# Sidharthshanu/Gossip-protocol-with-power-law

Measured on AMD Instinct MI355X. Metric: gossip edge-deliveries/s (GTEPS) & HBM roofline %, 2^24 nodes x 4096 msgs, higher is better.
Workload: dtype u64

## Files before the change

### gossip-protocol-with-power-law_amd/csrc/driver.hip

```cpp
#include <hip/hip_runtime.h>

#include <cstdlib>
#include <rccl/rccl.h>

#include <algorithm>
#include <cmath>
#include <cstring>
#include <string>
#include <vector>

#include "gp_device.h"
#include "xplan.h"

namespace gp {

static thread_local std::string g_err;
int set_error(int code, const std::string& msg) {
  g_err = msg;
  return code;
}
int copy_sync(Ctx* c, void* dst, const void* src, size_t bytes, hipMemcpyKind kind) {
  if (bytes == 0) return 0;
  GP_HIP(hipMemcpyAsync(dst, src, bytes, kind, c->stream));
  GP_HIP(hipStreamSynchronize(c->stream));
  return 0;
}

__global__ void k_stats_reduce(u64* __restrict__ partial, u64* __restrict__ stats) {
  __shared__ u64 acc[BLOCK];
  const int k = blockIdx.x;
  u64 t = 0;
  for (int p = threadIdx.x; p < NPART; p += BLOCK) {
    t += partial[(size_t)k * NPART + p];
    partial[(size_t)k * NPART + p] = 0;
  }
  acc[threadIdx.x] = t;
  __syncthreads();
  for (int w = BLOCK / 2; w > 0; w >>= 1) {
    if (threadIdx.x < w) acc[threadIdx.x] += acc[threadIdx.x + w];
    __syncthreads();
  }
  if (threadIdx.x == 0) stats[k] += acc[0];
}

__global__ __launch_bounds__(BLOCK) void k_mkbits(const uint32_t* __restrict__ fpop, u64* __restrict__ abits,
                                                  int64_t n, const uint32_t* __restrict__ seenpop,
                                                  const uint32_t* __restrict__ done_at, u64* __restrict__ dbits,
                                                  const uint8_t* __restrict__ sated,
                                                  const int32_t* __restrict__ deg_live, u64* __restrict__ partial) {
  const int lane = threadIdx.x & 63;
  const int64_t stride = (int64_t)gridDim.x * BLOCK;
  u64 sends = 0, active = 0;
  for (int64_t v0 = (int64_t)blockIdx.x * BLOCK + (threadIdx.x & ~63); v0 < n; v0 += stride) {
    const int64_t v = v0 + lane;
    const uint32_t fp = v < n ? fpop[v] : 0u;
    const u64 m = __ballot(fp != 0u);
    if (deg_live && fp) {
      sends += (u64)fp * (u64)(uint32_t)max(deg_live[v], 0);
      ++active;
    }
    if (lane == 0) abits[v0 >> 6] = m;
    if (dbits) {
      bool d = false;
      if (v < n) {
        if (sated) {
          const uint8_t sv = sated[v];
          const uint32_t t = done_at[v];
          d = !(sv & ST_DOWN) && ((sv & ST_SATED) || (t != 0u && seenpop[v] == t));
        } else {
          const uint32_t t = done_at[v];
          d = t != 0u && seenpop[v] == t;
        }
      }
      const u64 dm = __ballot(d);
      if (lane == 0) dbits[v0 >> 6] = dm;
    }
  }
  if (deg_live) {
    sends = wave_sum_u64(sends);
    active = wave_sum_u64(active);
    if (lane == 0) {
      const size_t p = blockIdx.x % NPART;
      if (sends) atomicAdd(&partial[(size_t)S_SENDS * NPART + p], sends);
      if (active) atomicAdd(&partial[(size_t)S_ACTIVE * NPART + p], active);
    }
  }
}

__global__ __launch_bounds__(BLOCK) void k_mksum(const u64* __restrict__ abits, u64* __restrict__ sbits,
                                                 int64_t nwords) {
  const int lane = threadIdx.x & 63;
  const int64_t k = (int64_t)blockIdx.x * WAVES + (threadIdx.x >> 6);
  const int64_t w = k * 64 + lane;
  const u64 m = __ballot(w < nwords && abits[w] != 0ull);
  if (lane == 0 && k * 64 < nwords) sbits[k] = m;
}

__global__ void k_lost_clear(const int32_t* __restrict__ origin, const u64* __restrict__ bits,
                             const uint32_t* __restrict__ cnt, const uint8_t* __restrict__ state,
                             const int32_t* __restrict__ midx, u64* __restrict__ cmask,
                             uint32_t* __restrict__ lostcnt, int64_t off, int64_t groups, int32_t words) {
  const int64_t t = (int64_t)blockIdx.x * blockDim.x + threadIdx.x;
  if (t >= groups * words) return;
  const int64_t gi = off + t / words;
  const int32_t w = (int32_t)(t % words);
  const int32_t o = origin[gi];
  if (!(state[o] & ST_DOWN)) return;
  const int32_t k = midx[o];
  atomicAnd(cmask + (size_t)k * words + w, ~bits[gi * words + w]);
  if (w == 0) atomicAdd(lostcnt + k, cnt[gi]);
}
__global__ void k_done_fix(const int32_t* __restrict__ midx, const uint32_t* __restrict__ lostcnt,
                           uint32_t* __restrict__ done_at, int64_t n) {
  for (int64_t v = (int64_t)blockIdx.x * blockDim.x + threadIdx.x; v < n; v += (int64_t)gridDim.x * blockDim.x) {
    const int32_t k = midx[v];
    if (k >= 0) {
      const uint32_t l = lostcnt[k];
      if (l) done_at[v] -= l;
    }
  }
}

struct InjectArgs {
  const int32_t* __restrict__ origin;
  const u64* __restrict__ bits;
  const uint32_t* __restrict__ cnt;
  u64* slot[2];
  int32_t rslot;
// ... 91 lines not shown
  static_assert(W <= 64, "W <= 64");
  constexpr int VPS = 64 / W;
  __shared__ uint32_t lc[CNT ? W * 64 : 1];
  __shared__ uint32_t lsum[SUM ? W * 64 : 1];
  for (int t = threadIdx.x; t < W * 64; t += BLOCK) {
    if (CNT) lc[t] = 0;
    if (SUM) lsum[t] = 0;
  }
  __syncthreads();
  const int lane = threadIdx.x & 63, wib = threadIdx.x >> 6;
  const int w = lane % W, q = lane / W;
  uint32_t c[64], s[64];
#pragma unroll
  for (int b = 0; b < 64; ++b) {
    c[b] = 0;
    s[b] = 0;
  }
  const int64_t step = (int64_t)gridDim.x * WAVES * VPS;
  for (int64_t i = ((int64_t)blockIdx.x * WAVES + wib) * VPS + q; i < a.count; i += step) {
    u64 x = 0;
    if (!a.guard || a.guard[i] != 0) {
      x = a.rows[i * W + w];
    }
    const uint32_t wt = SUM ? (uint32_t)max(a.weight[i], 0) : 0u;
#pragma unroll
    for (int b = 0; b < 64; ++b) {
      const uint32_t bit = (uint32_t)(x >> b) & 1u;
      if (CNT) c[b] += bit;
      if (SUM) s[b] += bit * wt;
    }
  }
#pragma unroll
  for (int b = 0; b < 64; ++b) {
#pragma unroll
    for (int st = W; st < 64; st <<= 1) {
      if (CNT) c[b] += __shfl_xor(c[b], st);
      if (SUM) s[b] += __shfl_xor(s[b], st);
    }
  }
  if (q == 0) {
#pragma unroll
    for (int b = 0; b < 64; ++b) {
      if (CNT && c[b]) atomicAdd(&lc[w * 64 + b], c[b]);
      if (SUM && s[b]) atomicAdd(&lsum[w * 64 + b], s[b]);
    }
  }
  __syncthreads();
  for (int t = threadIdx.x; t < W * 64; t += BLOCK) {
    if (CNT && lc[t]) atomicAdd(&a.cnt[t], (u64)lc[t]);
    if (SUM && lsum[t]) atomicAdd(&a.wsum[t], (u64)lsum[t]);
  }
}

int launch_activity_bits(Ctx* c, bool summary) {
  hipLaunchKernelGGL(k_mkbits, dim3(std::max(1, std::min(grid_for(c->n_alloc, BLOCK), c->cu_count * 8 * GS))),
                     dim3(BLOCK), 0, c->stream, c->d_fpop[c->cur], c->d_abits, c->n_alloc, c->d_seenpop,
                     c->d_done_at, (u64*)nullptr, (const uint8_t*)nullptr, (const int32_t*)nullptr, c->d_stats + 64);
  if (summary) {
    const int64_t nwords = (c->n_alloc + 63) / 64;
    hipLaunchKernelGGL(k_mksum, dim3(grid_for((nwords + 63) / 64, WAVES)), dim3(BLOCK), 0, c->stream, c->d_abits,
                       c->d_sbits, nwords);
  }
  GP_HIP(hipGetLastError());
  return 0;
}

static void fill_expand(Ctx* c, ExpandArgs& a) {
  const RoundPlan& p = c->plan;
  a.alive = alive_now(c) ? c->d_alive + (size_t)c->cur * c->words : nullptr;
  a.alive_next = alive_on(c) ? c->d_alive + (size_t)(c->cur ^ 1) * c->words : nullptr;
  a.row_ptr = c->d_row_ptr;
  a.col = c->d_col;
  a.rows = c->d_slot[c->cur];
  a.slot[0] = c->d_slot[0];
  a.slot[1] = c->d_slot[1];
  a.wslot = c->cur ^ 1;
  a.sp = c->d_sp;
  a.ws = c->d_ws;
  a.fpop = c->d_fpop[c->cur];
  a.abits = c->d_abits;
  a.sbits = p.sum ? c->d_sbits : nullptr;
  a.dbits = p.dnb ? c->d_dbits : nullptr;
  a.amask = c->d_amask;
  a.prehi = p.split ? c->d_prehi : nullptr;
  a.split_push = 0;
  a.acc_row = p.split ? c->acc_row : 0;
  a.lm = p.lines ? (c->carry.lm_written ? c->d_lmw[c->cur] : c->d_lm) : nullptr;
  a.lm_next = p.lm_write ? c->d_lmw[c->cur ^ 1] : nullptr;
  a.cmk = p.cml_read ? c->d_cmk[c->cur] : nullptr;
  a.cml = p.cml_read ? c->d_cml[c->cur] : nullptr;
  a.cmk_next = p.cml_write ? c->d_cmk[c->cur ^ 1] : nullptr;
  a.cml_next = p.cml_write ? c->d_cml[c->cur ^ 1] : nullptr;
  const bool frx_src = c->cfg.track_msg_forwards != 0 || c->local || c->rec[R_CURVE].want;
  a.frx = c->d_frx[0] && frx_src ? c->d_frx[c->cur] : nullptr;
  a.frx_next = c->d_frx[0] ? c->d_frx[c->cur ^ 1] : nullptr;
  a.frx_rows = c->frx_rows;
  a.done_at = c->d_done_at;
  a.gcol = c->d_gcol;
  a.midx = c->d_midx;
  a.cmask = c->d_cmask;
  a.unfiltered = p.unfiltered ? 1 : 0;
  a.near_done = p.near_done ? 1 : 0;
  a.sate = p.sate ? 1 : 0;
  a.ldone = p.line_done ? c->d_ldone : nullptr;
  a.early_exit = p.early_exit ? 1 : 0;
  a.dprobe = p.dprobe ? 1 : 0;
  a.alias = p.alias ? 1 : 0;
  a.ulist = p.ulist_read ? c->d_ulist[c->carry.ul_cur] : nullptr;
  a.ulist_n = p.ulist_read ? c->carry.ulist_n : 0;
  a.ulist_next = p.ulist_emit ? c->d_ulist[c->carry.ul_cur ^ 1] : nullptr;
// ... 38 lines not shown
  f.m = c->m;
  f.words = c->words;
  f.round = c->round;
  f.cfg = c->cfg;
  f.prev_new_bits = c->prev_new_bits;
  f.prev_receivers = c->prev_receivers;
  f.prev_next_arcs = c->prev_next_arcs;
  f.held_bits = c->held_bits;
  f.inj_arcs = (size_t)c->round < c->inj_arcs.size() ? (u64)c->inj_arcs[(size_t)c->round] : 0ull;
  f.inj_groups = c->inj_groups_at(c->round);
  f.last_inject_round = c->last_inject_round;
  f.local = c->local;
  f.liveness_active = c->liveness_active;
  f.alive_on = alive_on(c);
  f.alive_now = alive_now(c);
  f.have_cml = c->d_cml[0] != nullptr;
  f.have_lm = c->d_lm != nullptr;
  f.have_lmw = c->d_lmw[0] != nullptr;
  f.have_ldone = c->d_ldone != nullptr;
  f.have_ld_cand = c->n_ld_cand > 0;
  const int64_t row = c->words > 0 ? (int64_t)(c->d_acc - c->d_slot[c->cur]) / c->words : 0;
  f.acc_row = row > 0 && row + c->nloc() <= (int64_t)INT32_MAX ? row : 0;
  f.ld_env = c->ld_env;
  f.lp_env = c->lp_env;
  f.can_park = !c->carry.park_failed;
  f.carry = c->carry;
  f.lossy = c->loss_on || c->lag_on || c->repair_on;
  return f;
}

static int launch_expand(Ctx* c) {
  RoundFacts f = round_facts(c);
  RoundPlan p = plan_round(f);
  if (p.need_park_slot && !c->d_slot[2] && dalloc(&c->d_slot[2], (size_t)c->n_alloc * c->words) != 0) {
    (void)hipGetLastError();
    c->carry.park_failed = f.carry.park_failed = true;
    f.can_park = false;
    p = plan_round(f);
  }
  if (p.need_ulist && !c->d_ulist[0] &&
      (dalloc(&c->d_ulist[0], (size_t)c->n_alloc) != 0 || dalloc(&c->d_ulist[1], (size_t)c->n_alloc) != 0)) {
    dfree(&c->d_ulist[0]);
    dfree(&c->d_ulist[1]);
    (void)hipGetLastError();
    f.can_list = false;
    p = plan_round(f);
  }
  if (p.pull.kernel == PULL_LOSSY && (!c->d_frx[0] || c->frx_rows < c->n_alloc))
    return set_error(GP_ESTATE, "link loss is in force but the frontier rows are gone: gp_reset first");
  c->plan = p;
  c->acc_row = p.split ? (int32_t)f.acc_row : 0;
  if (alive_on(c))
    GP_HIP(hipMemsetAsync(c->d_alive + (size_t)(c->cur ^ 1) * c->words, 0, (size_t)c->words * 8, c->stream));
  if ((p.mode_push && c->nloc() > 0) || p.ulist_read || (p.pull.kernel == PULL_LOSSY && c->nloc() > 0))
    GP_HIP(hipMemsetAsync(c->d_fpop[c->cur ^ 1], 0, (size_t)c->nloc() * 4, c->stream));
  hipLaunchKernelGGL(k_mkbits, dim3(std::max(1, std::min(grid_for(c->n_alloc, BLOCK), c->cu_count * 8 * GS))),
                     dim3(BLOCK), 0, c->stream, c->d_fpop[c->cur], c->d_abits, c->n_alloc,
                     c->d_seenpop, c->d_done_at, p.dnb ? c->d_dbits : nullptr,
                     p.dnb && c->liveness_active ? (const uint8_t*)c->d_state : nullptr,
                     p.ulist_read ? (const int32_t*)c->d_deg_live : nullptr, c->d_stats + 64);
  if (c->carry.alias_active) {
    if (p.mode_push) GP_TRY(unalias(c, true));
    else if (!p.dprobe) GP_TRY(unalias(c, false));
  }
  if (p.sum) {
    const int64_t nwords = (c->n_alloc + 63) / 64;
    hipLaunchKernelGGL(k_mksum, dim3(grid_for((nwords + 63) / 64, WAVES)), dim3(BLOCK), 0, c->stream,
                       c->d_abits, c->d_sbits, nwords);
  }
  if (p.split) GP_TRY(build_prehi(c, c->cfg.split_deg));
  ExpandArgs a{};
  fill_expand(c, a);
  return launch_round_kernels(c, a);
}

template <int W>
static void launch_bitsum_w(Ctx* c, BitsumArgs a, bool cnt, bool sum) {
  const int grid = std::max(1, std::min(grid_for(a.count, (int64_t)WAVES * (64 / W)), c->cu_count * 2 * GS));
  if (cnt && sum)
    hipLaunchKernelGGL((k_bitsum<W, true, true>), dim3(grid), dim3(BLOCK), 0, c->stream, a);
  else if (cnt)
    hipLaunchKernelGGL((k_bitsum<W, true, false>), dim3(grid), dim3(BLOCK), 0, c->stream, a);
  else if (sum)
    hipLaunchKernelGGL((k_bitsum<W, false, true>), dim3(grid), dim3(BLOCK), 0, c->stream, a);
}

static int launch_bitsum(Ctx* c, BitsumArgs a, bool cnt, bool sum) {
  if (a.count <= 0) return 0;
  GP_TRY(with_words(c->words, [&](auto w) { launch_bitsum_w<w()>(c, a, cnt, sum); }));
  GP_HIP(hipGetLastError());
  return 0;
}

int bitsum_count_rows(Ctx* c, const u64* rows, const uint32_t* guard, int64_t count, u64* cnt) {
  BitsumArgs b{};
  b.rows = rows;
  b.guard = guard;
  b.cnt = cnt;
  b.count = count;
  return launch_bitsum(c, b, true, false);
}

static int round_launch(Ctx* c) {
  if (!state_ready(c) || c->words <= 0) return set_error(GP_ESTATE, "gp_set_messages + gp_reset first");
  if (c->round > 253) return set_error(GP_ESTATE, "round limit (254) reached");
  GP_TRY(lag_check_round(c));
  GP_TRY(repair_check_round(c));
  GP_HIP(hipSetDevice(c->device));
  hipStream_t s = c->stream;
  u64* stats = c->d_stats;
  u64* partial = c->d_stats + 64;
  const int r = c->round;
  lag_rotate(c);
  GP_HIP(hipMemsetAsync(stats, 0, 64 * sizeof(u64), s));
  GP_HIP(hipEventRecord(c->ev[0], s));
  if (c->liveness_active) {
    c->msg_forwards_valid = c->msg_forwards_valid && (c->cfg.track_msg_forwards != 0);
    GP_TRY(launch_liveness(c));
  }

  auto it = c->inject.find(r);
  if (it != c->inject.end() && it->second.cnt > 0) {
    GP_TRY(unalias(c, false));
    InjectArgs ia{};
    ia.origin = c->d_inj_origin;
    ia.bits = c->d_inj_bits;
    ia.cnt = c->d_inj_cnt;
    ia.slot[0] = c->d_slot[0];
    ia.slot[1] = c->d_slot[1];
    ia.rslot = c->cur;
    ia.sp = c->d_sp;
    ia.ws = c->d_ws;
    ia.fpop = c->d_fpop[c->cur];
    ia.frx = c->d_frx[0] ? c->d_frx[c->cur] : nullptr;
    ia.frx_rows = c->frx_rows;
    ia.cmk = c->d_cmk[0] ? c->d_cmk[c->cur] : nullptr;
    ia.alive = alive_on(c) ? c->d_alive + (size_t)c->cur * c->words : nullptr;
    ia.seenpop = c->d_seenpop;
    ia.first = c->cfg.track_first ? c->d_first : nullptr;
    ia.digest = c->cfg.track_digest ? c->d_digest : nullptr;
    ia.state = c->d_state;
    ia.lm = c->carry.lm_written ? c->d_lmw[c->cur] : nullptr;
    ia.partial = partial;
    ia.off = it->second.off;
    ia.groups = it->second.cnt;
    ia.vbegin = 0;
    ia.vend = c->nloc();
    ia.words = c->words;
    ia.wbase = c->cfg.msg_word_base;
    ia.r = r;
    hipLaunchKernelGGL(k_inject, dim3(grid_for(ia.groups, WAVES)), dim3(BLOCK), 0, s, ia);
    GP_HIP(hipGetLastError());
    if (c->liveness_active && c->cmask_rows > 0) {
      GP_HIP(hipMemsetAsync(c->d_lostcnt, 0, (size_t)c->cmask_rows * 4, s));
      hipLaunchKernelGGL(k_lost_clear, dim3(grid_for(ia.groups * c->words, 256)), dim3(256), 0, s,
                         c->d_inj_origin, c->d_inj_bits, c->d_inj_cnt, c->d_state, c->d_midx, c->d_cmask,
                         c->d_lostcnt, ia.off, ia.groups, c->words);
      hipLaunchKernelGGL(k_done_fix, dim3(std::min(grid_for(c->n_alloc, 256), c->cu_count * 8)), dim3(256), 0, s,
                         c->d_midx, c->d_lostcnt,
                         c->d_done_at, c->n_alloc);
      GP_HIP(hipGetLastError());
      c->done_dirty = true;
    }
  }

  if (c->cfg.track_msg_forwards) {
    BitsumArgs b{};
    b.rows = c->d_frx[c->cur];
    b.guard = c->d_fpop[c->cur];
    b.weight = c->d_deg_live;
    b.cnt = nullptr;
    b.wsum = c->d_msg_fwd;
    b.count = c->nloc();
    GP_TRY(launch_bitsum(c, b, false, true));
  }
  GP_TRY(load_before_expand(c));

  GP_HIP(hipEventRecord(c->ev[1], s));
  GP_TRY(launch_expand(c));
  hipLaunchKernelGGL(k_stats_reduce, dim3(NST), dim3(BLOCK), 0, s, partial, stats);
  GP_HIP(hipGetLastError());
  GP_HIP(hipEventRecord(c->ev[2], s));
  return records_count_round(c);
}

static int round_exchange_rccl(Ctx* c) {
  if (!c->comm) {
    if (c->local) return set_error(GP_ESTATE, "a partitioned context exchanges over RCCL (gp_comm_init) "
                                              "or in gp_round_group");
    return 0;
  }
  if (c->local) return exchange_rccl(c);
  GP_RCCL(ncclAllReduce(c->d_stats, c->d_stats, S_REPORT_CURSOR, ncclUint64, ncclSum, c->comm, c->stream));
  return 0;
}

static int round_collect(Ctx* c, gp_round_stats* out) {
  hipStream_t s = c->stream;
  const int r = c->round;
  GP_HIP(hipEventRecord(c->ev[3], s));
  GP_HIP(hipMemcpyAsync(c->h_stats, c->d_stats, 64 * sizeof(u64), hipMemcpyDeviceToHost, s));
  GP_HIP(hipStreamSynchronize(s));
  const u64* h = c->h_stats;
  if (h[S_XERR])
    return set_error(GP_ERCCL, "boundary exchange: " + std::to_string(h[S_XERR]) +
                                   " received entries do not match the exchange plan (round " + std::to_string(r) + ")");
  gp_round_stats own;
  {
    gp_round_stats* out = &own;
    std::memset(out, 0, sizeof(*out));
    out->round = r;
    out->injected = h[S_INJECTED];
    out->lost = h[S_LOST];
    out->new_bits = h[S_NEW_BITS];
    out->receivers = h[S_RECEIVERS];
    out->sends = h[S_SENDS];
    out->active = h[S_ACTIVE];
    out->crashed = h[S_CRASHED];
    out->reports = h[S_REPORTS];
    out->removals = h[S_REMOVALS];
    out->dup_reports = h[S_DUP];
    out->arcs_scanned = h[S_ARCS];
    out->rows_gathered = h[S_GATHERED];
    out->seen_rows_read = h[S_SEEN_READ];
    out->rows_written = h[S_WRITTEN];
    out->vertices_visited = h[S_VISITED];
    out->atomics = h[S_ATOMICS];
    out->next_arcs = h[S_NEXT_ARCS];
    out->row_bytes = h[S_ROW_BYTES];
    out->mode = c->plan.pull.kernel == PULL_LOSSY ? 2 : c->plan.mode_push ? 1 : 0;
    out->scan = c->plan.scan();
    out->kernel_ms = 0.0;
    if (!c->plan.mode_push && c->nloc() > 0) {
      float kms = 0.f;
      (void)hipEventElapsedTime(&kms, c->ev[4], c->ev[5]);
      out->kernel_ms = kms;
    }
    out->overflow = (int64_t)h[S_REPORT_CURSOR] > c->report_cap ? 1 : 0;
    out->xchg_rows = h[S_XROWS];
    out->xchg_bytes = h[S_XBYTES];
    out->done_nb = h[S_DNB];
    out->lm_rows = h[S_LM_ROWS];
    out->aliased = h[S_ALIASED];
    float ms = 0.f;
    (void)hipEventElapsedTime(&ms, c->ev[1], c->ev[2]);
    out->expand_ms = ms;
    (void)hipEventElapsedTime(&ms, c->ev[2], c->ev[3]);
    out->exchange_ms = ms;
    (void)hipEventElapsedTime(&ms, c->ev[0], c->ev[3]);
    out->round_ms = ms;
  }
  if (out) *out = own;
  c->run_stats.push_back(own);
  c->last_reports = (int64_t)h[S_REPORT_CURSOR];
  c->prev_next_arcs = h[S_NEXT_ARCS];
// ... 380 lines not shown
```

### gossip-protocol-with-power-law_amd/csrc/gp_internal.h

```cpp
#pragma once
#include <hip/hip_runtime.h>
#include <rccl/rccl.h>

#include <cstdint>
#include <map>
#include <string>
#include <type_traits>
#include <vector>

#include "../../include/gossip_capi.h"
#include "gp_common.h"
#include "records.h"
#include "round_plan.h"

namespace gp {

typedef unsigned long long u64;

enum StatSlot {
  S_INJECTED = 0, S_LOST, S_NEW_BITS, S_RECEIVERS, S_SENDS, S_ACTIVE, S_CRASHED,
  S_REPORTS, S_REMOVALS, S_DUP, S_ARCS, S_GATHERED, S_SEEN_READ, S_WRITTEN,
  S_VISITED, S_NEXT_ARCS, S_ATOMICS, S_ROW_BYTES,
  S_XROWS, S_XBYTES,
  S_DNB,
// ... 184 lines not shown
  u64* d_sbits = nullptr;
  u64* d_dbits = nullptr;
  uint8_t* d_lm = nullptr;
  uint8_t* d_lmw[2] = {nullptr, nullptr};
  int32_t* d_ulist[2] = {nullptr, nullptr};
  int32_t acc_row = 0;
  u64* d_amask = nullptr;
  u64* d_acc = nullptr;
  u64* d_tbits = nullptr;
  int32_t* d_touched = nullptr;
  int32_t* d_active = nullptr;
  int32_t* d_big = nullptr;
  std::vector<int64_t> inj_arcs;
  u64 prev_next_arcs = 0;
  u64 prev_new_bits = 0;
  u64 prev_receivers = 0;
  u64 held_bits = 0;
  u64* d_cml[2] = {nullptr, nullptr};
  u64* d_cmk[2] = {nullptr, nullptr};
  int64_t inj_groups_at(int32_t r) const {
    auto it = inject.find(r);
    return it == inject.end() ? 0 : it->second.cnt;
  }
  int32_t* d_gcol = nullptr;
  uint32_t* d_hub_done = nullptr;
  uint32_t hub_epoch = 0;
  int32_t* d_prehi = nullptr;
  int32_t prehi_deg = 0;
  int32_t* d_midx = nullptr;
  u64* d_cmask = nullptr;
  std::vector<int32_t> h_inj_origin;
  std::vector<u64> h_inj_bits;
  std::vector<int32_t> h_deg_out;
  uint32_t* d_done_at = nullptr;
  uint32_t* d_done_at0 = nullptr;
  u64* d_cmask0 = nullptr;
  uint32_t* d_lostcnt = nullptr;
  int32_t cmask_rows = 0;
  bool done_dirty = false;
  u64* d_msg_cov = nullptr;
  u64* d_msg_fwd = nullptr;
  u64* d_alive = nullptr;
  u64* d_bc_keys = nullptr;
  uint32_t* d_bc_part = nullptr;
  size_t bc_part_words = 0;
  int64_t bc_split = 0;
  u64* d_fin_comp = nullptr;
  u64* d_fin_list = nullptr;
  int32_t fin_comp_rows = 0;
  gp_report* d_reports = nullptr;
  int64_t report_cap = 0;
  u64* d_stats = nullptr;
  u64* h_stats = nullptr;
  int32_t round = 0;
  bool liveness_active = false;
  int32_t alive_from = -1;
  bool pending_crash = false;
  bool msg_forwards_valid = true;
  int64_t last_reports = 0;

  std::vector<HubItem> h_hub_items;
  HubItem* d_hub_items = nullptr;
  int32_t* d_hubs = nullptr;
  int32_t* d_hub_item_ptr = nullptr;
  u64* d_hub_partial = nullptr;
  uint32_t* d_hub_pnz = nullptr;
  int64_t n_hubs = 0, n_hub_items = 0;
  int32_t* d_border = nullptr;
  int32_t* d_ld_cand = nullptr;
  int64_t n_ld_cand = 0;
  uint8_t* d_ldone = nullptr;
  size_t ldone_bytes = 0;
  int32_t ld_env = -1;
  int32_t ld_min_deg = 0;
  int32_t lp_env = -1;

  ncclComm_t comm = nullptr;

  ncclComm_t jcomm = nullptr;
  gp_allgather_fn jhost = nullptr;
  void* jhost_user = nullptr;
  int32_t jrank = 0, jnranks = 0;
  u64* d_hist = nullptr;
  int32_t hist_cap = 0, hist_rounds = 0;
  int64_t hist_nw = 0;
  bool hist_valid = true;
  std::vector<gp_round_stats> run_stats;
  int32_t fin_round = -1;
  u64* d_jscr = nullptr;
  size_t jscr_words = 0;
  u64* d_jdig = nullptr;
  size_t jdig_words = 0;
  u64* d_jcf = nullptr;
  int32_t jm = 0;
  bool j_ready = false, j_fwd_valid = false, j_dig_valid = false;
  u64* d_jcurve = nullptr;
  size_t jcurve_words = 0;
  int32_t j_curve_rows = 0;
  bool j_curve_valid = false;

  int cu_count = 256;

  int64_t nloc() const { return vend - vbegin; }
  int64_t to_local(int64_t g) const;

};
// ... 112 lines not shown
```

### gossip-protocol-with-power-law_amd/csrc/setup.hip

```cpp
#include <cstdlib>
#include <cstring>
#include <string>
#include <vector>

#include "block_order.h"
#include "delay_planes.h"
#include "gp_device.h"
#include "line_cands.h"
#include "xplan.h"

namespace gp {

__device__ __forceinline__ int32_t cc_parent(const int32_t* p, int32_t x) {
  return __hip_atomic_load(p + x, __ATOMIC_RELAXED, __HIP_MEMORY_SCOPE_AGENT);
}
__device__ int32_t cc_find(int32_t* __restrict__ parent, int32_t x) {
  int32_t p = cc_parent(parent, x);
  while (p != x) {
    const int32_t g = cc_parent(parent, p);
    if (g != p) __hip_atomic_store(parent + x, g, __ATOMIC_RELAXED, __HIP_MEMORY_SCOPE_AGENT);
    x = p;
    p = g;
  }
  return x;
// ... 355 lines not shown

static int compute_done_at(Ctx* c, int64_t groups) {
  uint32_t* cnt = nullptr;
  GP_TRY(dalloc(&cnt, (size_t)c->n));
  hipStream_t s = c->stream;
  GP_HIP(hipMemsetAsync(cnt, 0, (size_t)c->n * 4, s));
  GP_HIP(hipMemsetAsync(c->d_done_at, 0, (size_t)c->n_alloc * 4, s));
  if (groups > 0)
    hipLaunchKernelGGL(k_count_origins, dim3(grid_for(groups, 256)), dim3(256), 0, s, c->d_inj_origin,
                       c->d_inj_cnt, groups, c->d_comp, cnt);
  hipLaunchKernelGGL(k_done_at, dim3(grid_for(c->n_alloc, 256)), dim3(256), 0, s, c->d_comp, cnt, c->d_done_at,
                     c->n_alloc);
  GP_HIP(hipGetLastError());
  GP_HIP(hipStreamSynchronize(s));
  dfree(&cnt);
  std::vector<int32_t> comp((size_t)c->n_alloc);
  GP_TRY(copy_sync(c, comp.data(), c->d_comp, (size_t)c->n_alloc * 4, hipMemcpyDeviceToHost));
  std::vector<int32_t> idx_of_root((size_t)c->n, -1);
  std::vector<u64> masks;
  const size_t W = (size_t)c->words;
  int32_t K = 0;
  for (int64_t g = 0; g < groups; ++g) {
    const int32_t root = comp[(size_t)c->h_inj_origin[(size_t)g]];
    if (idx_of_root[(size_t)root] < 0) {
      idx_of_root[(size_t)root] = K++;
      masks.resize((size_t)K * W, 0);
    }
    u64* row = masks.data() + (size_t)idx_of_root[(size_t)root] * W;
    for (size_t w = 0; w < W; ++w) row[w] |= c->h_inj_bits[(size_t)g * W + w];
  }
  if (masks.empty()) masks.assign(W, 0);
  GP_TRY(dalloc(&c->d_cmask, masks.size()));
  GP_TRY(copy_sync(c, c->d_cmask, masks.data(), masks.size() * 8, hipMemcpyHostToDevice));
  int32_t* ior = nullptr;
  GP_TRY(dalloc(&ior, (size_t)c->n));
  GP_TRY(copy_sync(c, ior, idx_of_root.data(), (size_t)c->n * 4, hipMemcpyHostToDevice));
  GP_TRY(dalloc(&c->d_midx, (size_t)c->n_alloc));
  GP_HIP(hipMemsetAsync(c->d_midx, 0xFF, (size_t)c->n_alloc * 4, s));
  hipLaunchKernelGGL(k_midx, dim3(grid_for(c->n_alloc, 256)), dim3(256), 0, s, c->d_comp, ior, c->d_midx,
                     c->n_alloc);
  GP_HIP(hipGetLastError());
  c->cmask_rows = (int32_t)(masks.size() / W);
  GP_TRY(dalloc(&c->d_cmask0, masks.size()));
  GP_TRY(dalloc(&c->d_done_at0, (size_t)c->n_alloc));
  GP_TRY(dalloc(&c->d_lostcnt, (size_t)c->cmask_rows));
  GP_HIP(hipMemcpyAsync(c->d_cmask0, c->d_cmask, masks.size() * 8, hipMemcpyDeviceToDevice, s));
  GP_HIP(hipMemcpyAsync(c->d_done_at0, c->d_done_at, (size_t)c->n_alloc * 4, hipMemcpyDeviceToDevice, s));
  c->done_dirty = false;
  GP_HIP(hipStreamSynchronize(s));
  dfree(&ior);
  return 0;
}


}

using namespace gp;

extern "C" {


void gp_default_config(gp_config* cfg) {
  if (!cfg) return;
  std::memset(cfg, 0, sizeof(*cfg));
  cfg->track_first = 0;
  cfg->track_digest = 1;
  cfg->track_msg_forwards = 0;
  cfg->churn = 0;
  cfg->p_fail = 0.0;
  cfg->churn_seed = 0;
  cfg->miss_threshold = 3;
  cfg->hub_threshold = 4096;
  cfg->report_capacity = 1 << 20;
  cfg->push_ratio = 100.0;
  cfg->early_exit = 1;
  cfg->arc_mask_permille = 0;
  cfg->prefilter_pct = 20;
  cfg->compact_rows = 0;
  cfg->unfiltered_pct = 90;
  cfg->msg_word_base = 0;
  cfg->flat_max_words = 16;
  cfg->summary_min_n = 1ll << 25;
  cfg->partition_by_arcs = 0;
#ifndef GP_SPLIT_DEG_DEFAULT
#define GP_SPLIT_DEG_DEFAULT 128
#endif
#ifndef GP_SPLIT_MAX_PERMILLE
#define GP_SPLIT_MAX_PERMILLE 10
#endif
  cfg->split_deg = GP_SPLIT_DEG_DEFAULT;
  cfg->split_max_permille = GP_SPLIT_MAX_PERMILLE;
}

int gp_create(int device, gp_ctx** out) {
  if (!out) return set_error(GP_EINVAL, "null out");
  *out = nullptr;
  int ndev = 0;
  GP_HIP(hipGetDeviceCount(&ndev));
  if (device < 0 || device >= ndev) return set_error(GP_EINVAL, "device index out of range");
  GP_HIP(hipSetDevice(device));
  gp_ctx* c = new gp_ctx();
  c->device = device;
  gp_default_config(&c->cfg);
  c->ld_min_deg = GP_LINE_DONE_MIN_DEG;
  if (const char* e = getenv("GP_LINE_DONE")) c->ld_env = e[0] == '1' ? 1 : e[0] == '0' ? 0 : -1;
  if (const char* e = getenv("GP_LINE_DONE_MIN_DEG")) {
    const long k = strtol(e, nullptr, 10);
    if (k >= 1 && k <= INT32_MAX) c->ld_min_deg = (int32_t)k;
  }
  if (const char* e = getenv("GP_LINE_PACK")) c->lp_env = e[0] == '1' ? 1 : e[0] == '0' ? 0 : -1;
  c->curve_grid = curve_env_grid();
  c->curve_yard = curve_env_yardstick();
  c->load_force = load_env_eager();
  c->fresh_gather = fresh_env_gather();
  c->delay_force_rows = delay_env_rows();
  c->fresh_curve_grid = fresh_curve_env_grid();
  hipDeviceProp_t prop;
  if (hipGetDeviceProperties(&prop, device) == hipSuccess) c->cu_count = prop.multiProcessorCount;
  if (hipStreamCreateWithFlags(&c->stream, hipStreamNonBlocking) != hipSuccess) {
    delete c;
    return set_error(GP_EHIP, "hipStreamCreate failed");
  }
  if (hipStreamCreateWithFlags(&c->side, hipStreamNonBlocking) != hipSuccess) {
    gp_destroy(c);
    return set_error(GP_EHIP, "hipStreamCreate failed");
  }
  for (auto& e : c->ev) (void)hipEventCreate(&e);
  if (hipEventCreateWithFlags(&c->ev_fork, hipEventDisableTiming) != hipSuccess ||
      hipEventCreateWithFlags(&c->ev_join, hipEventDisableTiming) != hipSuccess) {
    gp_destroy(c);
    return set_error(GP_EHIP, "hipEventCreate failed");
  }
  if (dalloc(&c->d_stats, 64 + (size_t)NPART * NST) != 0) {
    gp_destroy(c);
    return GP_ENOMEM;
  }
  (void)hipMemsetAsync(c->d_stats, 0, (64 + (size_t)NPART * NST) * sizeof(u64), c->stream);
  (void)hipStreamSynchronize(c->stream);
  (void)hipHostMalloc((void**)&c->h_stats, 64 * sizeof(u64), hipHostMallocDefault);
  *out = c;
  return 0;
}

void gp_destroy(gp_ctx* c) {
  if (!c) return;
  (void)hipSetDevice(c->device);
  if (c->stream) (void)hipStreamSynchronize(c->stream);
  if (c->side) (void)hipStreamSynchronize(c->side);
  if (c->comm) (void)ncclCommDestroy(c->comm);
  shard_free(c);
  lag_release(c);
  repair_free(c);
  dfree(&c->d_row_ptr); dfree(&c->d_col); dfree(&c->d_out_row_ptr); dfree(&c->d_out_col);
  dfree(&c->d_deg_out); dfree(&c->d_comp); dfree(&c->d_abits); dfree(&c->d_dbits); dfree(&c->d_lm); dfree(&c->d_lmw[0]); dfree(&c->d_lmw[1]); dfree(&c->d_sbits); dfree(&c->d_amask); dfree(&c->d_cml[0]); dfree(&c->d_cml[1]); dfree(&c->d_cmk[0]); dfree(&c->d_cmk[1]); dfree(&c->d_done_at);
  dfree(&c->d_done_at0); dfree(&c->d_cmask0); dfree(&c->d_lostcnt); dfree(&c->d_alive);
  dfree(&c->d_gcol); dfree(&c->d_prehi); dfree(&c->d_midx); dfree(&c->d_cmask);
  dfree(&c->d_tbits); dfree(&c->d_nbits); dfree(&c->d_touched); dfree(&c->d_active); dfree(&c->d_big);
  dfree(&c->d_inj_origin); dfree(&c->d_inj_bits); dfree(&c->d_inj_cnt);
  dfree(&c->d_slot[2]);
  free_rows(c);
  for (int k = 0; k < 2; ++k) { dfree(&c->d_frx[k]); dfree(&c->d_fpop[k]); }
  dfree(&c->d_sp); dfree(&c->d_ws); dfree(&c->d_ldone); dfree(&c->d_ld_cand);
  dfree(&c->d_ulist[0]); dfree(&c->d_ulist[1]);
  dfree(&c->d_seenpop); dfree(&c->d_first); dfree(&c->d_digest);
  records_free(c);
  dfree(&c->d_state); dfree(&c->d_miss); dfree(&c->d_deg_live); dfree(&c->d_cand);
  dfree(&c->d_det_big); dfree(&c->d_det_pre); dfree(&c->d_det_live); dfree(&c->d_det_cur); dfree(&c->d_det_base);
  dfree(&c->d_msg_cov); dfree(&c->d_reports); dfree(&c->d_stats);
  dfree(&c->d_hub_items); dfree(&c->d_hubs); dfree(&c->d_hub_item_ptr);
  dfree(&c->d_hub_partial); dfree(&c->d_hub_pnz); dfree(&c->d_hub_done); dfree(&c->d_border);
  bitcount_free(c);
  if (c->h_stats) (void)hipHostFree(c->h_stats);
  for (auto& e : c->ev) if (e) (void)hipEventDestroy(e);
  if (c->ev_fork) (void)hipEventDestroy(c->ev_fork);
  if (c->ev_join) (void)hipEventDestroy(c->ev_join);
  if (c->side) (void)hipStreamDestroy(c->side);
  if (c->stream) (void)hipStreamDestroy(c->stream);
  delete c;
}

int gp_configure(gp_ctx* c, const gp_config* cfg) {
  if (!c || !cfg) return set_error(GP_EINVAL, "null argument");
  if (cfg->p_fail < 0.0 || !(cfg->p_fail <= 1.0)) return set_error(GP_EINVAL, "p_fail must be in [0,1]");
  if (cfg->miss_threshold < 1 || cfg->miss_threshold > 254) return set_error(GP_EINVAL, "miss_threshold in [1,254]");
  if (cfg->hub_threshold < 64) return set_error(GP_EINVAL, "hub_threshold must be >= 64");
  if (cfg->report_capacity < 0) return set_error(GP_EINVAL, "report_capacity < 0");
  if (cfg->msg_word_base < 0) return set_error(GP_EINVAL, "msg_word_base < 0");
  if (cfg->prefilter_pct < 0) return set_error(GP_EINVAL, "prefilter_pct < 0");
  if (cfg->summary_min_n < 0) return set_error(GP_EINVAL, "summary_min_n < 0");
  if (cfg->compact_rows != 0 && cfg->compact_rows != 1) return set_error(GP_EINVAL, "compact_rows must be 0 or 1");
  if (cfg->arc_mask_permille < 0) return set_error(GP_EINVAL, "arc_mask_permille < 0");
  if (cfg->partition_by_arcs != 0 && cfg->partition_by_arcs != 1)
// ... 200 lines not shown
    std::vector<int64_t> rp(2);
    for (int32_t k = 0; k < m; ++k) {
      GP_TRY(copy_sync(c, rp.data(), c->d_row_ptr + origin[k], 2 * sizeof(int64_t), hipMemcpyDeviceToHost));
      keys[(size_t)k] = (u64)(rp[1] - rp[0]);
    }
  } else {
    int32_t* d_o = nullptr;
    u64 *d_k = nullptr, *d_s2 = nullptr;
    int rc = 0;
    if (hipMalloc(&d_o, (size_t)m * sizeof(int32_t)) != hipSuccess ||
        hipMalloc(&d_k, (size_t)m * sizeof(u64)) != hipSuccess)
      rc = set_error(GP_ENOMEM, "gp_spread_keys: message scratch");
    if (rc == 0) rc = copy_sync(c, d_o, origin, (size_t)m * sizeof(int32_t), hipMemcpyHostToDevice);
    if (rc == 0 && hops == 3 && hipMalloc(&d_s2, (size_t)c->n * sizeof(u64)) != hipSuccess)
      rc = set_error(GP_ENOMEM, "gp_spread_keys: n u64 of scratch");
    if (rc == 0) {
      if (hops == 3)
        hipLaunchKernelGGL(k_nbsum, dim3(std::min(grid_for(c->n, BLOCK / 64), 65536)), dim3(BLOCK), 0, c->stream,
                           c->d_row_ptr, c->d_col, (const u64*)nullptr, (const int32_t*)nullptr, c->n, d_s2);
      hipLaunchKernelGGL(k_nbsum, dim3(std::min(grid_for(m, BLOCK / 64), 65536)), dim3(BLOCK), 0, c->stream,
                         c->d_row_ptr, c->d_col, (const u64*)d_s2, (const int32_t*)d_o, (int64_t)m, d_k);
      if (hipGetLastError() != hipSuccess) rc = set_error(GP_EHIP, "gp_spread_keys: launch failed");
      if (rc == 0) rc = copy_sync(c, keys.data(), d_k, (size_t)m * sizeof(u64), hipMemcpyDeviceToHost);
    }
    if (d_o) (void)hipFree(d_o);
    if (d_k) (void)hipFree(d_k);
    if (d_s2) (void)hipFree(d_s2);
    if (rc) return rc;
  }
  std::memcpy(keys_out, keys.data(), (size_t)m * sizeof(u64));
  return 0;
}

int gp_reset(gp_ctx* c) {
  if (!c) return set_error(GP_EINVAL, "null ctx");
  GP_HIP(hipSetDevice(c->device));
  GP_TRY(lag_reset(c));
  GP_TRY(repair_check_reset(c));
  GP_TRY(loss_reset(c));
  if (!state_ready(c) || c->frx_sized != frx_users(c) || c->curve_alloc != c->rec[R_CURVE].want)
    GP_TRY(alloc_state(c));
  if (!c->done_at_valid) {
    GP_TRY(compute_done_at(c, c->n_groups));
    c->done_at_valid = true;
  } else if (c->done_dirty) {
    GP_HIP(hipMemcpyAsync(c->d_cmask, c->d_cmask0, (size_t)c->cmask_rows * c->words * 8,
                          hipMemcpyDeviceToDevice, c->stream));
    GP_HIP(hipMemcpyAsync(c->d_done_at, c->d_done_at0, (size_t)c->n_alloc * 4, hipMemcpyDeviceToDevice,
                          c->stream));
    c->done_dirty = false;
  }
  const size_t W = (size_t)c->words, na = (size_t)c->n_alloc, nl = (size_t)std::max<int64_t>(c->nloc(), 1);
  hipStream_t s = c->stream;
  GP_HIP(hipMemsetAsync(c->d_sp, SLOT_NONE, na, s));
  GP_HIP(hipMemsetAsync(c->d_ws, 0, na, s));
  GP_HIP(hipMemsetAsync(c->d_seenpop, 0, nl * 4, s));
  GP_HIP(hipMemsetAsync(c->d_fpop[0], 0, na * 4, s));
  GP_HIP(hipMemsetAsync(c->d_fpop[1], 0, na * 4, s));
  if (c->d_first) GP_HIP(hipMemsetAsync(c->d_first, 0xFF, nl * W * 64, s));
  GP_HIP(hipMemsetAsync(c->d_digest, 0, nl * 8, s));
  GP_HIP(hipMemsetAsync(c->d_state, 0, na, s));
  GP_HIP(hipMemsetAsync(c->d_tbits, 0, (na + 63) / 64 * 8, s));
  c->prev_next_arcs = 0;
  c->prev_new_bits = 0;
  c->prev_receivers = 0;
  c->held_bits = 0;
  c->carry = RoundCarry{};
  c->plan = RoundPlan{};
  GP_HIP(hipMemsetAsync(c->d_miss, 0, na, s));
  GP_HIP(hipMemsetAsync(c->d_deg_live, 0, na * 4, s));
  GP_HIP(hipMemcpyAsync(c->d_deg_live, c->d_deg_out, (size_t)c->n_alloc * 4, hipMemcpyDeviceToDevice, s));
  GP_HIP(hipMemsetAsync(c->d_msg_cov, 0, W * 64 * 4 * 8, s));
  GP_HIP(hipMemsetAsync(c->d_alive, 0, 2 * W * 8, s));
  GP_HIP(hipMemsetAsync(c->d_stats, 0, (64 + (size_t)NPART * NST) * 8, s));
  c->cur = 0;
  c->round = 0;
  c->liveness_active = c->cfg.churn != 0;
  c->alive_from = c->liveness_active ? 0 : -1;
  c->pending_crash = false;
  c->msg_forwards_valid = true;
  c->last_reports = 0;
  shard_reset(c);
  GP_TRY(records_reset(c));
  GP_TRY(lag_prepare(c));
  GP_TRY(repair_reset(c));
  GP_HIP(hipStreamSynchronize(s));
  return 0;
}

int gp_crash(gp_ctx* c, int32_t nverts, const int32_t* verts) {
  if (!c || (nverts > 0 && !verts)) return set_error(GP_EINVAL, "null argument");
  if (!state_ready(c)) return set_error(GP_ESTATE, "gp_reset first");
  GP_HIP(hipSetDevice(c->device));
  for (int32_t k = 0; k < nverts; ++k)
    if (verts[k] < 0 || verts[k] >= c->n) return set_error(GP_EINVAL, "vertex out of range");
  GP_TRY(unalias(c, false));
  if (nverts > 0 && !c->liveness_active) GP_TRY(load_before_liveness(c));
  std::vector<uint8_t> st((size_t)c->n_alloc);
  GP_HIP(hipStreamSynchronize(c->stream));
  GP_TRY(copy_sync(c, st.data(), c->d_state, (size_t)c->n_alloc, hipMemcpyDeviceToHost));
  for (int32_t k = 0; k < nverts; ++k) {
    const int64_t v = c->to_local(verts[k]);
    if (v >= 0 && !(st[(size_t)v] & ST_DOWN)) st[(size_t)v] |= ST_PENDING;
  }
  GP_TRY(copy_sync(c, c->d_state, st.data(), (size_t)c->n_alloc, hipMemcpyHostToDevice));
  if (nverts > 0) {
    if (!c->liveness_active) c->alive_from = c->round + 1;
    c->liveness_active = true;
    c->pending_crash = true;
  }
  return 0;
}

}
```

Before: 28730.

## Vectorize mkbits, fold next-frontier zeroing in, fuse reset memsets and stats readback

k_mkbits now has each lane handle four vertices through 16-byte vector loads, rebuilds the 64-bit activity and done masks with shuffles and ballots, and zeroes the next frontier population array inline in place of a separate memset. The per-round stats copy to the host becomes a tiny kernel that writes to pinned memory and clears the device stats, so the next round's memset can be skipped. gp_reset merges a dozen memsets and one copy into a single multi-segment kernel. The aim is fewer launches and API calls and better memory bandwidth, at the cost of more complex bit assembly and a reliance on alignment assumptions.

Result: no change. 28880 (median of 6 runs) (+0.5%).

```diff
diff --git a/gossip-protocol-with-power-law_amd/csrc/driver.hip b/gossip-protocol-with-power-law_amd/csrc/driver.hip
--- a/gossip-protocol-with-power-law_amd/csrc/driver.hip
+++ b/gossip-protocol-with-power-law_amd/csrc/driver.hip
@@ -43,37 +43,89 @@
   if (threadIdx.x == 0) stats[k] += acc[0];
 }
 
+__global__ void k_stats_out(u64* __restrict__ stats, u64* __restrict__ host) {
+  const int k = threadIdx.x;
+  host[k] = stats[k];
+  stats[k] = 0;
+}
+
+template <typename T>
+__device__ __forceinline__ void load_quad(const T* __restrict__ p, int64_t v, int64_t n, T (&x)[4]) {
+  struct alignas(4 * sizeof(T)) Quad { T e[4]; };
+  if (v + 4 <= n) {
+    const Quad q = *reinterpret_cast<const Quad*>(p + v);
+#pragma unroll
+    for (int k = 0; k < 4; ++k) x[k] = q.e[k];
+  } else {
+#pragma unroll
+    for (int k = 0; k < 4; ++k) x[k] = v + k < n ? p[v + k] : T(0);
+  }
+}
+__device__ __forceinline__ void store_quad_bits(u64* __restrict__ bits, int64_t v0, int64_t n, uint32_t nib, int lane) {
+  u64 mine = 0;
+#pragma unroll
+  for (int j = 0; j < 4; ++j) {
+    const uint32_t t = (uint32_t)__shfl((int)nib, 16 * j + (lane >> 2));
+    const u64 m = __ballot((t >> (lane & 3)) & 1u);
+    if (lane == j) mine = m;
+  }
+  if (lane < 4 && v0 + 64 * lane < n) bits[(v0 >> 6) + lane] = mine;
+}
 __global__ __launch_bounds__(BLOCK) void k_mkbits(const uint32_t* __restrict__ fpop, u64* __restrict__ abits,
                                                   int64_t n, const uint32_t* __restrict__ seenpop,
                                                   const uint32_t* __restrict__ done_at, u64* __restrict__ dbits,
                                                   const uint8_t* __restrict__ sated,
-                                                  const int32_t* __restrict__ deg_live, u64* __restrict__ partial) {
+                                                  const int32_t* __restrict__ deg_live, u64* __restrict__ partial,
+                                                  uint32_t* __restrict__ zero_next, int64_t nzero) {
   const int lane = threadIdx.x & 63;
-  const int64_t stride = (int64_t)gridDim.x * BLOCK;
+  const int64_t stride = (int64_t)gridDim.x * BLOCK * 4;
   u64 sends = 0, active = 0;
-  for (int64_t v0 = (int64_t)blockIdx.x * BLOCK + (threadIdx.x & ~63); v0 < n; v0 += stride) {
-    const int64_t v = v0 + lane;
-    const uint32_t fp = v < n ? fpop[v] : 0u;
-    const u64 m = __ballot(fp != 0u);
-    if (deg_live && fp) {
-      sends += (u64)fp * (u64)(uint32_t)max(deg_live[v], 0);
-      ++active;
-    }
-    if (lane == 0) abits[v0 >> 6] = m;
+  for (int64_t v0 = ((int64_t)blockIdx.x * BLOCK + (threadIdx.x & ~63)) * 4; v0 < n; v0 += stride) {
+    const int64_t v = v0 + 4 * lane;
+    uint32_t fp[4];
+    load_quad(fpop, v, n, fp);
+    uint32_t nib = 0;
+#pragma unroll
+    for (int k = 0; k < 4; ++k) nib |= (fp[k] != 0u ? 1u : 0u) << k;
+    if (zero_next) {
+      if (v + 4 <= nzero) {
+        *reinterpret_cast<uint4*>(zero_next + v) = uint4{0u, 0u, 0u, 0u};
+      } else {
+#pragma unroll
+        for (int k = 0; k < 4; ++k)
+          if (v + k < nzero) zero_next[v + k] = 0u;
+      }
+    }
+    if (deg_live && nib) {
+      int32_t dl[4];
+      load_quad(deg_live, v, n, dl);
+#pragma unroll
+      for (int k = 0; k < 4; ++k)
+        if (fp[k]) {
+          sends += (u64)fp[k] * (u64)(uint32_t)max(dl[k], 0);
+          ++active;
+        }
+    }
+    store_quad_bits(abits, v0, n, nib, lane);
     if (dbits) {
-      bool d = false;
+      uint32_t dnib = 0;
       if (v < n) {
+        uint32_t t[4], sn[4];
+        load_quad(done_at, v, n, t);
+        load_quad(seenpop, v, n, sn);
         if (sated) {
-          const uint8_t sv = sated[v];
-          const uint32_t t = done_at[v];
-          d = !(sv & ST_DOWN) && ((sv & ST_SATED) || (t != 0u && seenpop[v] == t));
+          uint8_t sv[4];
+          load_quad(sated, v, n, sv);
+#pragma unroll
+          for (int k = 0; k < 4; ++k)
+            if (v + k < n && !(sv[k] & ST_DOWN) && ((sv[k] & ST_SATED) || (t[k] != 0u && sn[k] == t[k]))) dnib |= 1u << k;
         } else {
-          const uint32_t t = done_at[v];
-          d = t != 0u && seenpop[v] == t;
+#pragma unroll
+          for (int k = 0; k < 4; ++k)
+            if (v + k < n && t[k] != 0u && sn[k] == t[k]) dnib |= 1u << k;
         }
       }
-      const u64 dm = __ballot(d);
-      if (lane == 0) dbits[v0 >> 6] = dm;
+      store_quad_bits(dbits, v0, n, dnib, lane);
     }
   }
   if (deg_live) {
@@ -271,10 +323,14 @@
   }
 }
 
+static int mkbits_grid(const Ctx* c) {
+  return std::max(1, std::min(grid_for(c->n_alloc, (int64_t)BLOCK * 4), c->cu_count * 8 * GS));
+}
+
 int launch_activity_bits(Ctx* c, bool summary) {
-  hipLaunchKernelGGL(k_mkbits, dim3(std::max(1, std::min(grid_for(c->n_alloc, BLOCK), c->cu_count * 8 * GS))),
-                     dim3(BLOCK), 0, c->stream, c->d_fpop[c->cur], c->d_abits, c->n_alloc, c->d_seenpop,
-                     c->d_done_at, (u64*)nullptr, (const uint8_t*)nullptr, (const int32_t*)nullptr, c->d_stats + 64);
+  hipLaunchKernelGGL(k_mkbits, dim3(mkbits_grid(c)), dim3(BLOCK), 0, c->stream, c->d_fpop[c->cur], c->d_abits,
+                     c->n_alloc, c->d_seenpop, c->d_done_at, (u64*)nullptr, (const uint8_t*)nullptr,
+                     (const int32_t*)nullptr, c->d_stats + 64, (uint32_t*)nullptr, (int64_t)0);
   if (summary) {
     const int64_t nwords = (c->n_alloc + 63) / 64;
     hipLaunchKernelGGL(k_mksum, dim3(grid_for((nwords + 63) / 64, WAVES)), dim3(BLOCK), 0, c->stream, c->d_abits,
@@ -419,13 +475,12 @@
   c->acc_row = p.split ? (int32_t)f.acc_row : 0;
   if (alive_on(c))
     GP_HIP(hipMemsetAsync(c->d_alive + (size_t)(c->cur ^ 1) * c->words, 0, (size_t)c->words * 8, c->stream));
-  if ((p.mode_push && c->nloc() > 0) || p.ulist_read || (p.pull.kernel == PULL_LOSSY && c->nloc() > 0))
-    GP_HIP(hipMemsetAsync(c->d_fpop[c->cur ^ 1], 0, (size_t)c->nloc() * 4, c->stream));
-  hipLaunchKernelGGL(k_mkbits, dim3(std::max(1, std::min(grid_for(c->n_alloc, BLOCK), c->cu_count * 8 * GS))),
-                     dim3(BLOCK), 0, c->stream, c->d_fpop[c->cur], c->d_abits, c->n_alloc,
-                     c->d_seenpop, c->d_done_at, p.dnb ? c->d_dbits : nullptr,
+  const bool zero_next = (p.mode_push && c->nloc() > 0) || p.ulist_read || (p.pull.kernel == PULL_LOSSY && c->nloc() > 0);
+  hipLaunchKernelGGL(k_mkbits, dim3(mkbits_grid(c)), dim3(BLOCK), 0, c->stream, c->d_fpop[c->cur], c->d_abits,
+                     c->n_alloc, c->d_seenpop, c->d_done_at, p.dnb ? c->d_dbits : nullptr,
                      p.dnb && c->liveness_active ? (const uint8_t*)c->d_state : nullptr,
-                     p.ulist_read ? (const int32_t*)c->d_deg_live : nullptr, c->d_stats + 64);
+                     p.ulist_read ? (const int32_t*)c->d_deg_live : nullptr, c->d_stats + 64,
+                     zero_next ? c->d_fpop[c->cur ^ 1] : (uint32_t*)nullptr, c->nloc());
   if (c->carry.alias_active) {
     if (p.mode_push) GP_TRY(unalias(c, true));
     else if (!p.dprobe) GP_TRY(unalias(c, false));
@@ -479,7 +534,8 @@
   u64* partial = c->d_stats + 64;
   const int r = c->round;
   lag_rotate(c);
-  GP_HIP(hipMemsetAsync(stats, 0, 64 * sizeof(u64), s));
+  if (!c->stats_clean) GP_HIP(hipMemsetAsync(stats, 0, 64 * sizeof(u64), s));
+  c->stats_clean = false;
   GP_HIP(hipEventRecord(c->ev[0], s));
   if (c->liveness_active) {
     c->msg_forwards_valid = c->msg_forwards_valid && (c->cfg.track_msg_forwards != 0);
@@ -566,8 +622,11 @@
   hipStream_t s = c->stream;
   const int r = c->round;
   GP_HIP(hipEventRecord(c->ev[3], s));
-  GP_HIP(hipMemcpyAsync(c->h_stats, c->d_stats, 64 * sizeof(u64), hipMemcpyDeviceToHost, s));
+  GP_HIP(hipSetDevice(c->device));
+  hipLaunchKernelGGL(k_stats_out, dim3(1), dim3(64), 0, s, c->d_stats, c->h_stats);
+  GP_HIP(hipGetLastError());
   GP_HIP(hipStreamSynchronize(s));
+  c->stats_clean = true;
   const u64* h = c->h_stats;
   if (h[S_XERR])
     return set_error(GP_ERCCL, "boundary exchange: " + std::to_string(h[S_XERR]) +
diff --git a/gossip-protocol-with-power-law_amd/csrc/gp_internal.h b/gossip-protocol-with-power-law_amd/csrc/gp_internal.h
--- a/gossip-protocol-with-power-law_amd/csrc/gp_internal.h
+++ b/gossip-protocol-with-power-law_amd/csrc/gp_internal.h
@@ -260,6 +260,7 @@
   int64_t report_cap = 0;
   u64* d_stats = nullptr;
   u64* h_stats = nullptr;
+  bool stats_clean = false;
   int32_t round = 0;
   bool liveness_active = false;
   int32_t alive_from = -1;
diff --git a/gossip-protocol-with-power-law_amd/csrc/setup.hip b/gossip-protocol-with-power-law_amd/csrc/setup.hip
--- a/gossip-protocol-with-power-law_amd/csrc/setup.hip
+++ b/gossip-protocol-with-power-law_amd/csrc/setup.hip
@@ -431,6 +431,34 @@
   return 0;
 }
 
+
+constexpr int RESET_SEGS = 13;
+struct ResetSeg {
+  void* dst;
+  const void* src;
+  size_t bytes;
+  uint32_t fill;
+};
+struct ResetArgs {
+  ResetSeg seg[RESET_SEGS];
+};
+__global__ __launch_bounds__(BLOCK) void k_reset_state(ResetArgs a) {
+  const size_t t0 = (size_t)blockIdx.x * BLOCK + threadIdx.x, stride = (size_t)gridDim.x * BLOCK;
+#pragma unroll
+  for (int k = 0; k < RESET_SEGS; ++k) {
+    const ResetSeg g = a.seg[k];
+    const size_t n16 = g.bytes / 16;
+    uint4* __restrict__ d = static_cast<uint4*>(g.dst);
+    const uint4* __restrict__ sr = static_cast<const uint4*>(g.src);
+    const uint4 f = {g.fill, g.fill, g.fill, g.fill};
+    for (size_t i = t0; i < n16; i += stride) d[i] = sr ? sr[i] : f;
+    const size_t rest = g.bytes - n16 * 16;
+    if (t0 < rest) {
+      const size_t b = n16 * 16 + t0;
+      static_cast<uint8_t*>(g.dst)[b] = sr ? static_cast<const uint8_t*>(g.src)[b] : (uint8_t)g.fill;
+    }
+  }
+}
 
 }
 
@@ -516,7 +544,11 @@
   }
   (void)hipMemsetAsync(c->d_stats, 0, (64 + (size_t)NPART * NST) * sizeof(u64), c->stream);
   (void)hipStreamSynchronize(c->stream);
-  (void)hipHostMalloc((void**)&c->h_stats, 64 * sizeof(u64), hipHostMallocDefault);
+  if (hipHostMalloc((void**)&c->h_stats, 64 * sizeof(u64), hipHostMallocDefault) != hipSuccess || !c->h_stats) {
+    c->h_stats = nullptr;
+    gp_destroy(c);
+    return set_error(GP_ENOMEM, "pinned stats block");
+  }
   *out = c;
   return 0;
 }
@@ -823,27 +855,36 @@
   }
   const size_t W = (size_t)c->words, na = (size_t)c->n_alloc, nl = (size_t)std::max<int64_t>(c->nloc(), 1);
   hipStream_t s = c->stream;
-  GP_HIP(hipMemsetAsync(c->d_sp, SLOT_NONE, na, s));
-  GP_HIP(hipMemsetAsync(c->d_ws, 0, na, s));
-  GP_HIP(hipMemsetAsync(c->d_seenpop, 0, nl * 4, s));
-  GP_HIP(hipMemsetAsync(c->d_fpop[0], 0, na * 4, s));
-  GP_HIP(hipMemsetAsync(c->d_fpop[1], 0, na * 4, s));
+  ResetArgs ra{};
+  int ns = 0;
+  const auto seg = [&](void* dst, const void* src, size_t bytes, uint32_t fill) {
+    ra.seg[ns++] = ResetSeg{dst, src, bytes, fill};
+  };
+  seg(c->d_sp, nullptr, na, 0x01010101u * SLOT_NONE);
+  seg(c->d_ws, nullptr, na, 0u);
+  seg(c->d_seenpop, nullptr, nl * 4, 0u);
+  seg(c->d_fpop[0], nullptr, na * 4, 0u);
+  seg(c->d_fpop[1], nullptr, na * 4, 0u);
+  seg(c->d_digest, nullptr, nl * 8, 0u);
+  seg(c->d_state, nullptr, na, 0u);
+  seg(c->d_tbits, nullptr, (na + 63) / 64 * 8, 0u);
+  seg(c->d_miss, nullptr, na, 0u);
+  seg(c->d_deg_live, c->d_deg_out, na * 4, 0u);
+  seg(c->d_msg_cov, nullptr, W * 64 * 4 * 8, 0u);
+  seg(c->d_alive, nullptr, 2 * W * 8, 0u);
+  seg(c->d_stats, nullptr, (64 + (size_t)NPART * NST) * 8, 0u);
+  static_assert(RESET_SEGS == 13, "gp_reset fills every segment of ResetArgs");
+  hipLaunchKernelGGL(k_reset_state, dim3(std::max(1, std::min(grid_for((int64_t)(na * 4 / 16), BLOCK), c->cu_count * 8 * GS))),
+                     dim3(BLOCK), 0, s, ra);
+  GP_HIP(hipGetLastError());
   if (c->d_first) GP_HIP(hipMemsetAsync(c->d_first, 0xFF, nl * W * 64, s));
-  GP_HIP(hipMemsetAsync(c->d_digest, 0, nl * 8, s));
-  GP_HIP(hipMemsetAsync(c->d_state, 0, na, s));
-  GP_HIP(hipMemsetAsync(c->d_tbits, 0, (na + 63) / 64 * 8, s));
   c->prev_next_arcs = 0;
   c->prev_new_bits = 0;
   c->prev_receivers = 0;
   c->held_bits = 0;
   c->carry = RoundCarry{};
   c->plan = RoundPlan{};
-  GP_HIP(hipMemsetAsync(c->d_miss, 0, na, s));
-  GP_HIP(hipMemsetAsync(c->d_deg_live, 0, na * 4, s));
-  GP_HIP(hipMemcpyAsync(c->d_deg_live, c->d_deg_out, (size_t)c->n_alloc * 4, hipMemcpyDeviceToDevice, s));
-  GP_HIP(hipMemsetAsync(c->d_msg_cov, 0, W * 64 * 4 * 8, s));
-  GP_HIP(hipMemsetAsync(c->d_alive, 0, 2 * W * 8, s));
-  GP_HIP(hipMemsetAsync(c->d_stats, 0, (64 + (size_t)NPART * NST) * 8, s));
+  c->stats_clean = true;
   c->cur = 0;
   c->round = 0;
   c->liveness_active = c->cfg.churn != 0;
```
